# AlibabaResearch/efficientteacher

Measured on AMD Instinct MI355X. Metric: SSOD images/sec (teacher+student step) YOLOv5l 640px, higher is better.
Workload: dtype bf16

## Files before the change

efficientteacher_amd/_lib.py:

```python
import ctypes
import os
from ctypes import c_char_p, c_double, c_float, c_int, c_int64, c_size_t, c_void_p

import torch

_HERE = os.path.dirname(os.path.abspath(__file__))
LIB_PATH = os.environ.get("ET_HIP_LIB") or os.path.join(_HERE, "libet_hip.so")

ET_F32, ET_BF16, ET_F16 = 0, 1, 2

P = c_void_p
SIGNATURES = {
    "et_build_arch": (c_char_p, []),
    "et_abi_version": (c_int, []),
    "et_nms_ssod_workspace_bytes": (c_int, [c_int, c_int, ctypes.POINTER(c_size_t)]),
    "et_nms_workspace_bytes": (c_int, [c_int, c_int, c_int, c_int, c_int, ctypes.POINTER(c_size_t)]),
    "et_nms": (c_int, [P, c_int, c_int, c_int, c_float, c_float, c_int, c_int, ctypes.c_uint64, ctypes.c_uint64, c_int,
                       c_float, c_int, P, P, P, P, P, c_size_t, P]),
    "et_nms_ssod": (c_int, [P, c_int, c_int, c_int, c_float, c_float, c_int, c_int, P, P, P, P, P, c_size_t, P]),
    "et_val_match": (c_int, [P, c_int, P, c_int, c_int, P, c_int, P, c_int, c_int, P, c_int, c_int, c_int, c_int64, c_int64,
                             P, P, P, P, P, P]),
    "et_val_confusion": (c_int, [P, c_int, P, c_int, c_int, P, c_int, P, c_int, c_int, c_float, c_float, c_int, c_int, P, P]),
    "et_val_predn": (c_int, [P, c_int, P, c_int, c_int, P, c_int, c_int, c_int, P, P, P]),
    "et_val_ap_workspace_bytes": (c_int, [c_int, ctypes.POINTER(c_size_t)]),
# ... 37 lines not shown
                              c_size_t, P]),
    "et_bn_act_bwd_from_partials": (c_int, [P, c_int, P, c_int, P, c_int, c_int, c_int, c_int, P, P, P, P, P, c_int, P, P, P,
                                            P, c_int, P, P]),
    "et_act_bwd": (c_int, [P, c_int, P, c_int, P, c_int, c_int, c_int, c_int, c_int, P]),
    "et_pack_input": (c_int, [P, P, c_int, c_int, c_int, c_int, c_int, P]),
    "et_pack_input_u8": (c_int, [P, P, c_int, c_int, c_int, c_int, c_int, c_float, P]),
    "et_maxpool5_fwd": (c_int, [P, c_int, P, c_int, P, c_int, c_int, c_int, c_int, c_int, P]),
    "et_maxpool5_bwd": (c_int, [P, c_int, P, P, c_int, P, c_int, c_int, c_int, c_int, c_int, c_int, P]),
    "et_upsample2x_fwd": (c_int, [P, c_int, P, c_int, c_int, c_int, c_int, c_int, c_int, P]),
    "et_upsample2x_bwd": (c_int, [P, c_int, P, c_int, c_int, c_int, c_int, c_int, c_int, c_int, P]),
    "et_strong_view_u8": (c_int, [P, P, c_int, c_int, c_int, P, P, P, P, c_int, P]),
    "et_mosaic4_u8": (c_int, [P, P, c_int, c_int, c_int, P]),
    "et_pseudo_label_transform": (c_int, [P, P, P, c_int, c_int, c_int, c_int, c_int, P, P, P]),
    "et_score_log_append": (c_int, [P, P, c_int, c_int, P, P, P, c_int64, P]),
    "et_yolo_loss": (c_int, [P, P]),
    "et_ota_workspace_bytes": (c_int, [c_int, c_int, c_int, c_int, ctypes.POINTER(c_size_t)]),
    "et_ota_assign": (c_int, [P, P, c_float, c_int, P, P, P]),
    "et_select_targets": (c_int, [P, P, c_int, P, P, c_int, c_int, P, P]),
    "et_scale_cast": (c_int, [P, P, c_int, c_int64, c_float, P, P]),
    "et_domain_focal": (c_int, [P, c_int, c_int, c_int64, c_int, c_float, P, c_int, P, P]),
    "et_scale_inplace": (c_int, [P, c_int, c_int64, c_float, P, P]),
    "et_v8_decode": (c_int, [P, c_int, P, c_int, c_int, c_int, c_int, c_int, c_int, c_int, c_float, c_float, P, c_int64, c_int64, P]),
    "et_tal_loss": (c_int, [P, P, P, P, P, P, P, c_int, c_int, c_int, c_int, c_int, c_float, c_float, c_float, P, P, P, P, P]),
    "et_tal_assign_workspace_bytes": (c_int, [c_int, c_int, c_int, ctypes.POINTER(c_size_t)]),
    "et_tal_assign": (c_int, [P, P, P, P, P, P, c_int, c_int, c_int, c_int, c_int, c_float, c_float, c_float, P, P, P, P, P, c_size_t, P]),
    "et_tal_targets_pad": (c_int, [P, c_int, c_int, c_int, c_float, c_float, P, P, P]),
    "et_tal_pseudo_split": (c_int, [P, P, P, P, c_int, c_int, c_int, c_int, c_int, c_int, c_float, c_float, P, P, P, P, P, P, P, P, P]),
    "et_tal_assigned_gt": (c_int, [P, c_int, c_int, c_int, P, P]),
    "et_tal_merge_pseudo": (c_int, [P, P, P, P, P, P, P, P, P, c_int, c_int, c_int, c_int, P, P, P, P]),
}
# ... 132 lines not shown
```

efficientteacher_amd/autograd.py:

```python
import torch
from torch.autograd import Function

from . import ops

ACT_CODE = {"silu": ops.ACT_SILU, "relu": ops.ACT_RELU, "none": ops.ACT_NONE}

FUSE_BN_BWD = True
FUSE_BN_BWD_K = 1
_RS_DGRAD = {}


def _dgrad_on_rs_tile(cs, x):
    key = (tuple(x.shape), x.dtype, cs.cinp, cs.coutp, cs.k, cs.stride, cs.pad)
    r = _RS_DGRAD.get(key)
    if r is None:
        N, H, W, _ = x.shape
        r = _RS_DGRAD[key] = cs.stride == 1 and ops.kernel_name("dgrad_full", x.dtype, N, H, W, cs.cinp, cs.coutp, cs.k, cs.stride,
                                                               cs.pad).startswith("conv_gemm_rs_kernel")
    return r


def _fuse_into(cs, bn, x=None):
    if bn is None:
        return None
# ... 274 lines not shown
        dx = None
        if ctx.x_needs_grad:
            wf = cs1.w_lp.as_strided((2 * c, 1, 1, cs1.cinp), (cs1.cinp, cs1.cinp, cs1.cinp, 1), cs1.w_lp.storage_offset())
            dx = ops.conv2d_dgrad(dy, ops.weight_transpose(wf), (x.shape[1], x.shape[2]), 1, 0)
        return (dx,) + (None,) * 11


class _GradDst:

    def __init__(self, p):
        self.shape, self.stride, self.dtype, self.device = tuple(p.shape), tuple(p.stride()), p.dtype, p.device
        self.span = ops._flat_span(p)
        self.buf = None
        self.written = [False, False]

    def flat(self, half, n):
        if self.buf is None:
            self.buf = torch.empty(self.span, dtype=self.dtype, device=self.device)
        cut = n * self.stride[0]
        self.written[half] = True
        return self.buf[:cut] if half == 0 else self.buf[cut:]


class BatchSplitFn(Function):
    @staticmethod
    def forward(ctx, p, n, holder):
        ctx.n, ctx.holder = n, holder
        return p[:n], p[n:]

    @staticmethod
# ... 203 lines not shown
```

efficientteacher_amd/csrc/loss.hip:

```cpp
#include "et_device.h"
#include "../../include/et_hip.h"

#define LOSS_NPASS 4
#define LOSS_MAXL 4

struct LossLevel {
    const void* p;
    float* dp;
    unsigned long long* tobj;
    long long sb, sa, sy, sx;
    int ny, nx;
    float anchors[3][2];
    float balance;
};

struct LossArgs {
    int dtype, B, na, nc, no, NT, nl;
    float anchor_t, gr, cp, cn, cls_pw, obj_pw, box_w, obj_w, cls_w;
    int pass_mask;
    int ignore_obj;
    float* balance_dev;
    int ssi;
    float fl_gamma;
    int obj_ch;
// ... 222 lines not shown
                }
#pragma unroll
                for (int i = 0; i < 4; ++i) sg[i] = 1.0f / (1.0f + expf(-lg[i]));
                pb[0] = sg[0] * 2.f - 0.5f; pb[1] = sg[1] * 2.f - 0.5f;
                const float tw = sg[2] * 2, th = sg[3] * 2;
                pb[2] = tw * tw * L.anchors[r.a][0]; pb[3] = th * th * L.anchors[r.a][1];
                const float ciou = ciou_fwd_bwd(pb, r.tb, g);
                box_sum = 1.0f - ciou;
                const float wgt = -A.box_w / npos;
                atomicAdd(L.dp + off + 0, wgt * g[0] * 2.f * sg[0] * (1.f - sg[0]));
                atomicAdd(L.dp + off + 1, wgt * g[1] * 2.f * sg[1] * (1.f - sg[1]));
                atomicAdd(L.dp + off + 2, wgt * g[2] * L.anchors[r.a][0] * 8.f * sg[2] * sg[2] * (1.f - sg[2]));
                atomicAdd(L.dp + off + 3, wgt * g[3] * L.anchors[r.a][1] * 8.f * sg[3] * sg[3] * (1.f - sg[3]));
                if (pass == 0) {
                    const float tv = (1.0f - A.gr) + A.gr * fmaxf(ciou, 0.f);
                    atomicMax(L.tobj + cell, ((unsigned long long)r.seq << 32) | __float_as_uint(tv));
                }
            }
            if (pass == 1) {
                const float tv = A.ignore_obj ? -1.0f : r.score;
                atomicMax(L.tobj + cell, ((unsigned long long)r.seq << 32) | __float_as_uint(tv));
            }
            if (want_cls) {
                do_cls = true;
                cls_off = off;
                cls_c = r.c;
                cls_wgt = A.cls_w / (npos * (float)A.nc);
            }
        }
    }
    if (A.dtype == ET_F32) cls_sum += loss_class_walk<float>(A, L, do_cls, cls_off, cls_c, cls_wgt);
    else if (A.dtype == ET_F16) cls_sum += loss_class_walk<et_f16>(A, L, do_cls, cls_off, cls_c, cls_wgt);
    else cls_sum += loss_class_walk<uint16_t>(A, L, do_cls, cls_off, cls_c, cls_wgt);
    box_sum = et_wave_sum(box_sum);
    cls_sum = et_wave_sum(cls_sum);
    if ((threadIdx.x & 63) == 0) {
        if (box_sum != 0.f) atomicAdd(A.acc + level * 16 + ACC_BOX0 + pass, box_sum);
        if (cls_sum != 0.f) atomicAdd(A.acc + level * 16 + ACC_CLS0 + pass, cls_sum);
    }
}

__global__ __launch_bounds__(256) void loss_obj_kernel(LossArgs A, LossLevels Ls, int mode) {
    const int level = blockIdx.z;
    const LossLevel& L = Ls.l[level];
    const float fixed_n = Ls.fixed_n[level];
    const unsigned ncell = (unsigned)A.B * A.na * L.ny * L.nx;
    const unsigned plane = (unsigned)L.nx * L.ny;
    float lsum = 0.f, cnt = 0.f;
    const float n = (mode == 1) ? (fixed_n > 0.f ? fixed_n : A.acc[level * 16 + ACC_OBJN]) : 1.f;
    const float bal = (mode == 1) ? (A.balance_dev ? A.balance_dev[level] : L.balance) : 0.f;
    if (blockIdx.x * 256u >= ncell) return;
    for (unsigned i = blockIdx.x * 256u + threadIdx.x; i < ncell; i += gridDim.x * 256u) {
        const unsigned long long w = L.tobj[i];
        const float t = w ? __uint_as_float((unsigned)(w & 0xffffffffull)) : 0.0f;
        if (t >= 0.0f) {
            cnt += 1.f;
            if (mode == 1) {
                const unsigned q = i / plane, rem = i - q * plane;
                const unsigned gj = rem / (unsigned)L.nx, gi = rem - gj * (unsigned)L.nx;
                const unsigned b = q / (unsigned)A.na, a = q - b * (unsigned)A.na;
                const long long off = (long long)b * L.sb + (long long)a * L.sa + (long long)gj * L.sy + (long long)gi * L.sx + A.obj_ch;
                const float x = ld_logit(L.p, A.dtype, off);
                float g;
                lsum += focal_bce_logits(x, t, A.obj_pw, A.fl_gamma, g);
                L.dp[off] += g * (A.obj_w * bal / n);
            }
        }
    }
    __shared__ float red[2][4];
    lsum = et_wave_sum(lsum);
    cnt = et_wave_sum(cnt);
    if ((threadIdx.x & 63) == 0) { red[0][threadIdx.x >> 6] = lsum; red[1][threadIdx.x >> 6] = cnt; }
    __syncthreads();
    if (threadIdx.x == 0) {
        if (mode == 1) atomicAdd(A.acc + level * 16 + ACC_OBJ, red[0][0] + red[0][1] + red[0][2] + red[0][3]);
        else atomicAdd(A.acc + level * 16 + ACC_OBJN, red[1][0] + red[1][1] + red[1][2] + red[1][3]);
    }
}

__global__ void loss_finalize_kernel(LossArgs A, float b0, float b1, float b2, float b3, long long n0, long long n1,
// ... 13 lines not shown
                if ((p == 0 || p == 3) && A.nc > 1) lcls += a[ACC_CLS0 + p] / (n * (float)A.nc);
            }
        }
        const float nobj = A.ignore_obj ? a[ACC_OBJN] : (float)ncell[l];
        const float obji = a[ACC_OBJ] / nobj;
        lobj += obji * (A.balance_dev ? A.balance_dev[l] : bal[l]);
        if (A.balance_dev && A.ssi >= 0) A.balance_dev[l] = A.balance_dev[l] * 0.9999f + 0.0001f / obji;
    }
    if (A.balance_dev && A.ssi >= 0) {
        const float ref = A.balance_dev[A.ssi];
        for (int l = 0; l < A.nl; ++l) A.balance_dev[l] = A.balance_dev[l] / ref;
    }
    lbox *= A.box_w; lobj *= A.obj_w; lcls *= A.cls_w;
    out[0] = lbox; out[1] = lobj; out[2] = lcls;
    out[3] = (lbox + lobj + lcls) * (float)A.B;
}

#define OTA_K 13

struct OtaArgs {
    LossArgs A;
    LossLevel L[LOSS_MAXL];
    float stride[LOSS_MAXL];
    float img_size;
    int topk;
    int* order;
    int* istart;
    float* cbox;
    float* cs0;
    long long* coff;
// ... 243 lines not shown
    if (d->dtype != ET_F32 && d->dtype != ET_BF16 && d->dtype != ET_F16) return -2;
    const long long nq = (long long)d->nl * 5 * d->na * d->NT;
    if (nq >= (1ll << 31)) return -2;
    if (d->NT == 0) return 0;
    hipStream_t s = (hipStream_t)stream;
    OtaArgs O;
    LossArgs& A = O.A;
    A.dtype = d->dtype; A.B = d->B; A.na = d->na; A.nc = d->nc; A.no = d->nc + 5; A.NT = d->NT; A.nl = d->nl;
    A.anchor_t = d->anchor_t; A.gr = d->gr; A.cp = d->cp; A.cn = d->cn; A.cls_pw = d->cls_pw; A.obj_pw = d->obj_pw;
    A.box_w = d->box_w; A.obj_w = d->obj_w; A.cls_w = d->cls_w;
    A.pass_mask = 1; A.ignore_obj = 0; A.obj_ch = 4; A.ota_match = nullptr; A.fl_gamma = 0.f; A.balance_dev = nullptr; A.ssi = -1;
    A.tgt = d->targets; A.acc = nullptr;
    for (int l = 0; l < LOSS_MAXL; ++l) {
        LossLevel& L = O.L[l];
        O.stride[l] = 0.f;
        L.p = nullptr; L.dp = nullptr; L.tobj = nullptr; L.sb = L.sa = L.sy = L.sx = 0; L.ny = L.nx = 1; L.balance = 0.f;
        for (int a = 0; a < 3; ++a) L.anchors[a][0] = L.anchors[a][1] = 1.f;
        if (l >= d->nl) continue;
        const et_loss_level* e = &d->level[l];
        if (!e->p) return -1;
        L.p = e->p; L.sb = e->sb; L.sa = e->sa; L.sy = e->sy; L.sx = e->sx; L.ny = e->ny; L.nx = e->nx;
        for (int a = 0; a < d->na; ++a) { L.anchors[a][0] = e->anchors[2 * a]; L.anchors[a][1] = e->anchors[2 * a + 1]; }
        O.stride[l] = strides[l];
    }
    O.img_size = img_size; O.topk = top_k;
    char* w = (char*)workspace;
    O.coff = (long long*)w;  w += sizeof(long long) * nq;
    O.cbox = (float*)w;      w += sizeof(float) * 4 * nq;
    O.cs0 = (float*)w;       w += sizeof(float) * nq;
    O.cimg = (int*)w;        w += sizeof(int) * nq;
    O.cnt = (int*)w;         w += sizeof(int) * nq;
// ... 49 lines not shown
    const float f = dev_scale ? scale * dev_scale[0] : scale;
    if (i < n) d[i] = et_elem<T>::st(s[i] * f);
}

template <typename T = uint16_t>
__global__ __launch_bounds__(256) void scale_cast_bf16_vec8_kernel(const float* __restrict__ s, T* __restrict__ d, long long n8,
                                                                   float scale, const float* __restrict__ dev_scale) {
    const long long i = (long long)blockIdx.x * 256 + threadIdx.x;
    if (i >= n8) return;
    const float f = dev_scale ? scale * dev_scale[0] : scale;
    const float4 a = *(const float4*)(s + i * 8), b = *(const float4*)(s + i * 8 + 4);
    *(uint4*)(d + i * 8) = make_uint4(et_lp<T>::pack(a.x * f, a.y * f), et_lp<T>::pack(a.z * f, a.w * f), et_lp<T>::pack(b.x * f, b.y * f),
                                      et_lp<T>::pack(b.z * f, b.w * f));
}

extern "C" int et_yolo_loss(const et_loss_desc* d, et_stream_t stream) {
    if (!d || !d->targets || !d->acc_ws || !d->out) return -1;
    if (d->nl < 1 || d->nl > LOSS_MAXL || d->na < 1 || d->na > 3 || d->nc < 1 || d->NT < 0) return -2;
    if ((long long)5 * d->na * d->NT >= (1ll << 27)) return -2;
    hipStream_t s = (hipStream_t)stream;
    LossArgs A;
    A.dtype = d->dtype; A.B = d->B; A.na = d->na; A.nc = d->nc; A.no = d->nc + 5; A.NT = d->NT; A.nl = d->nl;
    A.anchor_t = d->anchor_t; A.gr = d->gr; A.cp = d->cp; A.cn = d->cn; A.cls_pw = d->cls_pw; A.obj_pw = d->obj_pw;
    A.box_w = d->box_w; A.obj_w = d->obj_w; A.cls_w = d->cls_w;
    A.pass_mask = d->pass_mask; A.ignore_obj = d->ignore_obj;
    A.ota_match = d->ota_match; A.obj_ch = d->obj_channel ? d->obj_channel : 4;
    A.fl_gamma = d->fl_gamma;
    A.balance_dev = d->balance_dev; A.ssi = d->balance_dev ? d->autobalance_ssi : -1;
    if (A.balance_dev && A.ssi >= A.nl) return -2;
    if (A.obj_ch < 4 || A.obj_ch >= A.no) return -2;
    A.tgt = d->targets; A.acc = d->acc_ws;
    if (A.dtype != ET_F32 && A.dtype != ET_BF16 && A.dtype != ET_F16) return -2;
    (void)hipMemsetAsync(d->acc_ws, 0, sizeof(float) * 16 * LOSS_MAXL, s);
    float bal[4] = {0, 0, 0, 0};
    long long ncell[4] = {0, 0, 0, 0};
    LossLevels Ls;
    long long ob_max = 1;
    for (int l = 0; l < d->nl; ++l) {
        const et_loss_level* e = &d->level[l];
        if (!e->p || !e->dp || !e->tobj_ws) return -1;
        LossLevel& L = Ls.l[l];
        L.p = e->p; L.dp = e->dp; L.tobj = (unsigned long long*)e->tobj_ws;
        L.sb = e->sb; L.sa = e->sa; L.sy = e->sy; L.sx = e->sx; L.ny = e->ny; L.nx = e->nx;
        for (int a = 0; a < d->na; ++a) { L.anchors[a][0] = e->anchors[2 * a]; L.anchors[a][1] = e->anchors[2 * a + 1]; }
        L.balance = e->balance;
        bal[l] = e->balance;
        ncell[l] = (long long)d->B * d->na * e->ny * e->nx;
        if (ncell[l] >= (1ll << 31)) return -2;
        Ls.fixed_n[l] = d->ignore_obj ? 0.f : (float)ncell[l];
        const long long ob = et_cdiv(ncell[l], 256);
        ob_max = ob > ob_max ? ob : ob_max;
        (void)hipMemsetAsync(e->tobj_ws, 0, (size_t)ncell[l] * 8, s);
    }
    for (int l = d->nl; l < LOSS_MAXL; ++l) { Ls.l[l] = Ls.l[0]; Ls.fixed_n[l] = 0.f; }
    const int nslot = 5 * d->na * d->NT;
    if (nslot > 0) {
        const dim3 grid((nslot + 255) / 256, LOSS_NPASS, d->nl);
        hipLaunchKernelGGL(loss_count_kernel, grid, dim3(256), 0, s, A, Ls);
        hipLaunchKernelGGL(loss_pos_kernel, grid, dim3(256), 0, s, A, Ls);
    }
    const dim3 og((unsigned)(ob_max < 512 ? ob_max : 512), 1, d->nl);
    if (d->ignore_obj) hipLaunchKernelGGL(loss_obj_kernel, og, dim3(256), 0, s, A, Ls, 0);
    hipLaunchKernelGGL(loss_obj_kernel, og, dim3(256), 0, s, A, Ls, 1);
    hipLaunchKernelGGL(loss_finalize_kernel, dim3(1), dim3(64), 0, s, A, bal[0], bal[1], bal[2], bal[3], ncell[0], ncell[1],
                       ncell[2], ncell[3], d->out);
    ET_CHECK_LAUNCH();
    return 0;
}

extern "C" int et_select_targets(const double* targets9, const uint8_t* valid, int N, const double* thr_low,
                                 const double* thr_high, int nc, int with_obj, float* table, et_stream_t stream) {
    if (!targets9 || !thr_low || !thr_high || !table) return -1;
    if (N < 0 || nc < 1) return -2;
    if (N == 0) return 0;
    hipLaunchKernelGGL(select_targets_kernel, dim3((N + 255) / 256), dim3(256), 0, (hipStream_t)stream, targets9, valid, N,
                       thr_low, thr_high, nc, with_obj, table);
    ET_CHECK_LAUNCH();
    return 0;
}

// ... 83 lines not shown
```

efficientteacher_amd/models/loss/loss.py:

```python
import torch

from ... import ops
from ...utils.torch_utils import is_parallel


def smooth_BCE(eps=0.1):
    return 1.0 - 0.5 * eps, 0.5 * eps


class YoloLossFn(torch.autograd.Function):

    @staticmethod
    def forward(ctx, table, hp, anchors_host, balance, *p):
        hp = dict(hp)
        ctx.grad_dst = hp.pop("grad_dst", None) or [None] * len(p)
        ota = hp.pop("ota", None)
        if ota is None:
            out, dps = ops.yolo_loss(list(p), table, anchors_host, balance, **hp)
        else:
            pl = list(p)
            match = ops.ota_assign(pl, table, anchors_host, ota["strides"], nc=hp["nc"], anchor_t=hp["anchor_t"],
                                   top_k=ota["top_k"], img_size=ota["img_size"])
            o1, dps = ops.yolo_loss(pl, table, anchors_host, balance, ota_match=match, obj_channel=hp["nc"] + 4, **hp)
            o2, dps = ops.yolo_loss(pl, table, anchors_host, balance, dps=dps, **hp)
            out = o1 + o2
        ctx.dps = dps
        ctx.meta = [(pi.shape, pi.stride(), pi.dtype) for pi in p]
        ctx.bs = p[0].shape[0]
        ctx.mark_non_differentiable()
        return out

    @staticmethod
    def backward(ctx, gout):
        g3 = gout[3:4].contiguous().float()
        grads = []
        for dp, (shape, stride, dtype), dst in zip(ctx.dps, ctx.meta, ctx.grad_dst):
            out = None
            if dst is not None:
                holder, half, n = dst
                flat = holder.flat(half, n)
                if flat.numel() == dp.numel() and holder.dtype == dtype:
                    out = flat
            g = ops.scale_cast(dp, dtype, scale=float(ctx.bs), dev_scale=g3, out=out)
            grads.append(g.as_strided(shape, stride))
        return (None, None, None, None, *grads)


def _head_of(model):
    return model.module.head if is_parallel(model) else model.head

# ... 81 lines not shown
```

efficientteacher_amd/ops.py:

```python
import torch

from . import _lib
from ._lib import ET_BF16, ET_F16, ET_F32

ACT_NONE, ACT_SILU, ACT_RELU = 0, 1, 2


class KernelTimer:

    def __init__(self):
        self.rows = []
        self.shapes = []

    def span(self, tag, flops, launches=1, nbytes=0, shape=None):
        a, b = torch.cuda.Event(enable_timing=True), torch.cuda.Event(enable_timing=True)
        self.rows.append((tag, flops, launches, nbytes, a, b))
        self.shapes.append(shape)
        return a, b

    def summary(self):
        agg = {}
        for tag, fl, n, nb, a, b in self.rows:
            ms = a.elapsed_time(b)
            t = agg.setdefault(tag, dict(ms=0.0, flops=0.0, launches=0, bytes=0.0))
            t["ms"] += ms; t["flops"] += fl; t["launches"] += n; t["bytes"] += nb
        return agg


TIMER = None
SCOPE = None


class FamilyTimer:

    FAMILY = {
        "et_conv2d_fwd": "gather_gemm", "et_conv2d_dgrad": "gather_gemm", "et_conv2d_dgrad_bn": "gather_gemm",
        "et_conv2d_wgrad": "wgrad", "et_conv2d_wgrad_grouped": "wgrad", "et_conv2d_stem_u8_fwd": "gather_gemm", "et_conv2d_stem_u8_wgrad": "wgrad",
        "et_bn_finalize": "bn", "et_bn_act_fwd": "bn", "et_bn_act_fwd_sharded": "bn", "et_bn_act_bwd_sharded": "bn", "et_bn_act_bwd": "bn", "et_bn_act_bwd_from_partials": "bn", "et_act_bwd": "bn",
        "et_nms": "nms_loss_pl", "et_nms_ssod": "nms_loss_pl", "et_detect_decode": "nms_loss_pl", "et_pseudo_label_transform": "nms_loss_pl",
        "et_select_targets": "nms_loss_pl", "et_yolo_loss": "nms_loss_pl", "et_ota_assign": "nms_loss_pl", "et_score_log_append": "nms_loss_pl",
        "et_scale_cast": "nms_loss_pl", "et_domain_focal": "nms_loss_pl", "et_scale_inplace": "nms_loss_pl", "et_v8_decode": "nms_loss_pl",
        "et_tal_loss": "nms_loss_pl", "et_tal_assign": "nms_loss_pl", "et_colsum": "nms_loss_pl", "et_tal_pseudo_split": "nms_loss_pl", "et_tal_targets_pad": "nms_loss_pl",
        "et_tal_assigned_gt": "nms_loss_pl", "et_tal_merge_pseudo": "nms_loss_pl",
        "et_sgd_nesterov": "optimizer_ema", "et_sgd_nesterov_dev": "optimizer_ema", "et_adamw": "optimizer_ema", "et_ema_update": "optimizer_ema",
        "et_ema_update_dev": "optimizer_ema", "et_cast_f32_to_lp": "optimizer_ema", "et_scaler_check": "optimizer_ema", "et_scaler_update": "optimizer_ema", "et_weight_transpose": "optimizer_ema",
        "et_weight_transpose_all": "optimizer_ema", "et_bn_eval_affine": "optimizer_ema",
    }

    def __init__(self):
        self.rows = []

    def begin(self, name):
        fam = self.FAMILY.get(name, "pool_upsample_pack")
        if fam == "gather_gemm":
            fam = "gather_gemm_teacher" if SCOPE == "teacher" else "gather_gemm_student"
# ... 836 lines not shown
        assert balance_dev.dtype == torch.float32 and balance_dev.numel() >= len(p) and balance_dev.device == dev
        d.balance_dev = _lib.ptr(balance_dev); d.autobalance_ssi = int(ssi)
    keep, new_dps = [table, acc], []
    for i, pi in enumerate(p):
        _, _, ny, nx, _ = pi.shape
        dp = dps[i] if dps is not None else torch.zeros(_flat_span(pi), dtype=torch.float32, device=dev)
        assert dp.numel() == _flat_span(pi)
        tobj = torch.empty(B * na * ny * nx, dtype=torch.int64, device=dev)
        L = d.level[i]
        L.dp = _lib.ptr(dp); L.tobj_ws = _lib.ptr(tobj)
        new_dps.append(dp); keep.append(tobj)
    _lib.check(lib.et_yolo_loss(ctypes.byref(d), _lib.stream(p[0])), "et_yolo_loss")
    return out, new_dps


def ota_assign(p, table, anchors_host, strides, *, nc, anchor_t, top_k=13, img_size=640.0):
    import ctypes
    lib = _lib.load()
    dev = p[0].device
    B, na, nl, NT = p[0].shape[0], p[0].shape[1], len(p), int(table.shape[0])
    table = table.contiguous()
    hp = dict(nc=nc, anchor_t=anchor_t, gr=1.0, cp=1.0, cn=0.0, cls_pw=1.0, obj_pw=1.0, box_w=0.0, obj_w=0.0, cls_w=0.0)
    d = _loss_desc(p, table, anchors_host, [0.0] * nl, hp, 1, False)
    match = torch.full((nl * 5 * na * NT,), -1, dtype=torch.int32, device=dev)
    if NT == 0:
        return match
    d.targets = _lib.ptr(table)
    nbytes = ctypes.c_size_t(0)
    _lib.check(lib.et_ota_workspace_bytes(B, na, nl, NT, ctypes.byref(nbytes)), "et_ota_workspace_bytes")
    ws = torch.empty(nbytes.value, dtype=torch.uint8, device=dev)
# ... 232 lines not shown
```

efficientteacher_amd/trainer/graph_step.py:

```python
import torch

from .. import ops


class HostStager:

    def __init__(self, n, device, slots=8, dtype=torch.float32):
        self.dev = torch.zeros(n, dtype=dtype, device=device)
        self.host = [torch.zeros(n, dtype=dtype).pin_memory() for _ in range(slots)]
        self.ev = [None] * slots
        self.i = 0

    def push(self, values):
        k = self.i % len(self.host)
        self.i += 1
        if self.ev[k] is not None:
            self.ev[k].synchronize()
        h = self.host[k]
        h.copy_(values if torch.is_tensor(values) else torch.as_tensor(values, dtype=h.dtype))
        self.dev.copy_(h, non_blocking=True)
        e = torch.cuda.Event()
        e.record()
        self.ev[k] = e
        return self.dev
# ... 38 lines not shown
            import torch.distributed as dist
            from ..parallel import FlatDataParallel
            if not (isinstance(t.model, FlatDataParallel) and dist.is_initialized() and dist.get_backend(t.model.pg) == "nccl"):
                return False
        if type(t.compute_loss).__name__ != "ComputeLoss":
            return False
        from ..optim import FlatSGD
        opt = t.optimizer
        if not isinstance(opt, FlatSGD) or opt.first:
            return False
        if targets.shape[0] > self.TARGET_CAPACITY:
            return False
        if self.graph is not None and self._signature(imgs) != self.sig:
            torch.cuda.synchronize(t.device)
            self.graph, self.items = None, None
            self.recaptures += 1
        return True

    def _capture(self, imgs, u_str, u_ori, M_s):
        t = self.t
        dev = t.device
        opt = t.optimizer
        emas = [e for e in (t.ema, t.semi_ema) if e is not None]
        self.hp = HostStager(4 * len(opt.param_groups) + 2 * len(emas), dev)
        opt.hp_dev = self.hp.dev[:4 * len(opt.param_groups)].view(len(opt.param_groups), 4)
        for i, e in enumerate(emas):
            e.d_dev = self.hp.dev[4 * len(opt.param_groups) + 2 * i:4 * len(opt.param_groups) + 2 * i + 2]
        self.emas = emas
        self.s_imgs, self.s_ustr, self.s_uori = imgs, u_str, u_ori
        self.s_M = M_s.to(device=dev, dtype=torch.float64).contiguous()
        self.tbl = HostStager(self.TARGET_CAPACITY * 8, dev, slots=4)
        self.s_table = self.tbl.dev.view(self.TARGET_CAPACITY, 8)
        self.hp.push(self._scalars(advance=False))
        torch.cuda.synchronize(dev)
        g = torch.cuda.CUDAGraph()
        for e in emas:
            e.capturing = True
        t._capturing = True
        opt.capturing = True
        import gc
        gc_was_on = gc.isenabled()
        gc.disable()
        try:
            with torch.cuda.graph(g, capture_error_mode="thread_local" if t.RANK != -1 else "global"):
                self.items = t._train_instance_eager(self.s_imgs, None, None, self.s_ustr, self.s_uori, None, self.s_M, 0,
                                                     sup_table=self.s_table)
        finally:
            if gc_was_on:
                gc.enable()
            t._capturing = False
            opt.capturing = False
            for e in emas:
                e.capturing = False
        self.graph = g
        self.sig = self._signature(imgs)
        self._probe, self._since_capture, self.probe_ms = [], 0, None

    def _check_probe(self):
        t = self.t
        self._probe[-1][1].synchronize()
        ms = sorted(a.elapsed_time(b) for a, b in self._probe)
        self.probe_ms = ms[len(ms) // 2]
        self._probe = []
        eager = t.eager_step_ms()
        if eager is None or self.probe_ms <= self.slow_factor * eager:
            return True
        self.slow_captures += 1
        torch.cuda.synchronize(t.device)
        self.graph, self.items = None, None
        if self.slow_captures >= 2:
            raise SlowReplay(f"captured step replays in {self.probe_ms:.1f} ms, the eager step takes {eager:.1f} ms (twice)")
        self.recaptures += 1
        return True

    def _scalars(self, advance=True):
        vals = self.t.optimizer.hp_values()
        for e in self.emas:
            d = e.advance() if advance else 0.5
            vals += [float(d), float(1. - d)]
        return vals

    def run(self, imgs, targets, u_str, u_ori, M_s, ni):
        t = self.t
        if self.graph is not None and len(self._probe) == self.REPLAY_PROBE:
# ... 40 lines not shown
```

include/et_hip.h:

```cpp
#ifndef ET_HIP_H
#define ET_HIP_H
#include <stddef.h>
#include <stdint.h>

#ifdef __cplusplus
extern "C" {
#endif

typedef void* et_stream_t;

enum { ET_F32 = 0, ET_BF16 = 1, ET_F16 = 2 };

#define ET_ABI_VERSION 9
const char* et_build_arch(void);
int et_abi_version(void);

int et_nms_ssod_workspace_bytes(int B, int A, size_t* bytes );
int et_nms_ssod(const float* pred, int B, int A, int no, float conf_thres, float iou_thres,
                int agnostic, int max_det, float* dets, int* counts, int64_t* keep,
                int* n_candidates, void* workspace, size_t ws_bytes, et_stream_t stream);

int et_nms_workspace_bytes(int B, int A, int no, int multi_label, int max_nms, size_t* bytes );
int et_nms(const float* pred, int B, int A, int no, float conf_thres, float iou_thres, int agnostic,
           int multi_label, uint64_t class_mask_lo, uint64_t class_mask_hi, int max_nms, float max_wh,
           int max_det, float* dets, int* counts, int64_t* keep, int* n_candidates, void* workspace,
           size_t ws_bytes, et_stream_t stream);

int et_val_match(const float* dets, int det_row_stride, const int* counts, int B, int max_det, const float* targets, int NT,
// ... 138 lines not shown
typedef struct {
    int dtype, B, na, nc, NT, nl;
    float anchor_t, gr, cp, cn, cls_pw, obj_pw, box_w, obj_w, cls_w;
    int pass_mask, ignore_obj;
    const float* targets;
    float* acc_ws;
    float* out;
    const int* ota_match;
    int obj_channel;
    float* balance_dev;
    int autobalance_ssi;
    float fl_gamma;
    et_loss_level level[4];
} et_loss_desc;
int et_yolo_loss(const et_loss_desc* desc , et_stream_t stream);
int et_ota_workspace_bytes(int B, int na, int nl, int NT, size_t* bytes);
int et_ota_assign(const et_loss_desc* desc , const float* strides , float img_size, int top_k,
                  void* workspace, int* match, et_stream_t stream);
int et_select_targets(const double* targets9, const uint8_t* valid, int N, const double* thr_low,
                      const double* thr_high, int nc, int with_obj, float* table, et_stream_t stream);
int et_scale_cast(const float* src, void* dst, int dtype, int64_t n, float scale,
                  const float* dev_scale , et_stream_t stream);

int et_domain_focal(const void* feat, int ldf, int dtype, int64_t P, int label, float gscale, void* grad,
                    int ldg, float* loss_sum, et_stream_t stream);
int et_scale_inplace(void* x, int dtype, int64_t n, float alpha, const float* dev_scale ,
                     et_stream_t stream);

int et_v8_decode(const void* reg, int ld_reg, const void* cls, int ld_cls, int dtype, int B, int H, int W, int reg_max, int nc,
                 float stride, float cell_offset, float* out, int64_t A_total, int64_t a_offset, et_stream_t stream);
// ... 26 lines not shown
```

Measured before the change: 1311.

## Use pooled sparse loss workspaces and emit dense grads in backward

Result: no change. 1319, median of 6 (+0.6%).

```diff
diff --git a/efficientteacher_amd/_lib.py b/efficientteacher_amd/_lib.py
--- a/efficientteacher_amd/_lib.py
+++ b/efficientteacher_amd/_lib.py
@@ -75,6 +75,8 @@
     "et_pseudo_label_transform": (c_int, [P, P, P, c_int, c_int, c_int, c_int, c_int, P, P, P]),
     "et_score_log_append": (c_int, [P, P, c_int, c_int, P, P, P, c_int64, P]),
     "et_yolo_loss": (c_int, [P, P]),
+    "et_yolo_loss_ws": (c_int, [P, P, P, P]),
+    "et_yolo_loss_emit": (c_int, [P, P, P, P, c_int, c_float, P, P]),
     "et_ota_workspace_bytes": (c_int, [c_int, c_int, c_int, c_int, ctypes.POINTER(c_size_t)]),
     "et_ota_assign": (c_int, [P, P, c_float, c_int, P, P, P]),
     "et_select_targets": (c_int, [P, P, c_int, P, P, c_int, c_int, P, P]),
diff --git a/efficientteacher_amd/autograd.py b/efficientteacher_amd/autograd.py
--- a/efficientteacher_amd/autograd.py
+++ b/efficientteacher_amd/autograd.py
@@ -312,6 +312,10 @@
         self.buf = None
         self.written = [False, False]
 
+    def span_of(self, half, n):
+        cut = n * self.stride[0]
+        return cut if half == 0 else self.span - cut
+
     def flat(self, half, n):
         if self.buf is None:
             self.buf = torch.empty(self.span, dtype=self.dtype, device=self.device)
diff --git a/efficientteacher_amd/csrc/loss.hip b/efficientteacher_amd/csrc/loss.hip
--- a/efficientteacher_amd/csrc/loss.hip
+++ b/efficientteacher_amd/csrc/loss.hip
@@ -3,11 +3,14 @@
 
 #define LOSS_NPASS 4
 #define LOSS_MAXL 4
+#define LOSS_TOUCHED (1ull << 63)
 
 struct LossLevel {
     const void* p;
     float* dp;
     unsigned long long* tobj;
+    float* gobj;
+    unsigned char* mark;
     long long sb, sa, sy, sx;
     int ny, nx;
     float anchors[3][2];
@@ -260,14 +263,17 @@
                 atomicAdd(L.dp + off + 3, wgt * g[3] * L.anchors[r.a][1] * 8.f * sg[3] * sg[3] * (1.f - sg[3]));
                 if (pass == 0) {
                     const float tv = (1.0f - A.gr) + A.gr * fmaxf(ciou, 0.f);
-                    atomicMax(L.tobj + cell, ((unsigned long long)r.seq << 32) | __float_as_uint(tv));
+                    atomicMax(L.tobj + cell, LOSS_TOUCHED | ((unsigned long long)r.seq << 32) | __float_as_uint(tv));
+                } else {
+                    atomicOr(L.tobj + cell, LOSS_TOUCHED);
                 }
             }
             if (pass == 1) {
                 const float tv = A.ignore_obj ? -1.0f : r.score;
-                atomicMax(L.tobj + cell, ((unsigned long long)r.seq << 32) | __float_as_uint(tv));
+                atomicMax(L.tobj + cell, LOSS_TOUCHED | ((unsigned long long)r.seq << 32) | __float_as_uint(tv));
             }
             if (want_cls) {
+                if (pass == 3) atomicOr(L.tobj + cell, LOSS_TOUCHED);
                 do_cls = true;
                 cls_off = off;
                 cls_c = r.c;
@@ -297,8 +303,14 @@
     const float bal = (mode == 1) ? (A.balance_dev ? A.balance_dev[level] : L.balance) : 0.f;
     if (blockIdx.x * 256u >= ncell) return;
     for (unsigned i = blockIdx.x * 256u + threadIdx.x; i < ncell; i += gridDim.x * 256u) {
-        const unsigned long long w = L.tobj[i];
+        const unsigned long long wt = L.tobj[i];
+        const unsigned long long w = wt & ~LOSS_TOUCHED;
         const float t = w ? __uint_as_float((unsigned)(w & 0xffffffffull)) : 0.0f;
+        if (mode == 1 && L.gobj) {
+            L.mark[i] = wt ? 1 : 0;
+            if (wt) L.tobj[i] = 0ull;
+            if (!(t >= 0.0f)) L.gobj[i] = 0.f;
+        }
         if (t >= 0.0f) {
             cnt += 1.f;
             if (mode == 1) {
@@ -309,7 +321,8 @@
                 const float x = ld_logit(L.p, A.dtype, off);
                 float g;
                 lsum += focal_bce_logits(x, t, A.obj_pw, A.fl_gamma, g);
-                L.dp[off] += g * (A.obj_w * bal / n);
+                if (L.gobj) L.gobj[i] = g * (A.obj_w * bal / n);
+                else L.dp[off] += g * (A.obj_w * bal / n);
             }
         }
     }
@@ -353,6 +366,7 @@
     lbox *= A.box_w; lobj *= A.obj_w; lcls *= A.cls_w;
     out[0] = lbox; out[1] = lobj; out[2] = lcls;
     out[3] = (lbox + lobj + lcls) * (float)A.B;
+    for (int i = 0; i < 16 * LOSS_MAXL; ++i) A.acc[i] = 0.f;
 }
 
 #define OTA_K 13
@@ -626,7 +640,7 @@
     for (int l = 0; l < LOSS_MAXL; ++l) {
         LossLevel& L = O.L[l];
         O.stride[l] = 0.f;
-        L.p = nullptr; L.dp = nullptr; L.tobj = nullptr; L.sb = L.sa = L.sy = L.sx = 0; L.ny = L.nx = 1; L.balance = 0.f;
+        L.p = nullptr; L.dp = nullptr; L.tobj = nullptr; L.gobj = nullptr; L.mark = nullptr; L.sb = L.sa = L.sy = L.sx = 0; L.ny = L.nx = 1; L.balance = 0.f;
         for (int a = 0; a < 3; ++a) L.anchors[a][0] = L.anchors[a][1] = 1.f;
         if (l >= d->nl) continue;
         const et_loss_level* e = &d->level[l];
@@ -706,7 +720,7 @@
                                       et_lp<T>::pack(b.z * f, b.w * f));
 }
 
-extern "C" int et_yolo_loss(const et_loss_desc* d, et_stream_t stream) {
+static int yolo_loss_run(const et_loss_desc* d, float* const* gobj, unsigned char* const* mark, et_stream_t stream) {
     if (!d || !d->targets || !d->acc_ws || !d->out) return -1;
     if (d->nl < 1 || d->nl > LOSS_MAXL || d->na < 1 || d->na > 3 || d->nc < 1 || d->NT < 0) return -2;
     if ((long long)5 * d->na * d->NT >= (1ll << 27)) return -2;
@@ -723,16 +737,16 @@
     if (A.obj_ch < 4 || A.obj_ch >= A.no) return -2;
     A.tgt = d->targets; A.acc = d->acc_ws;
     if (A.dtype != ET_F32 && A.dtype != ET_BF16 && A.dtype != ET_F16) return -2;
-    (void)hipMemsetAsync(d->acc_ws, 0, sizeof(float) * 16 * LOSS_MAXL, s);
+    if (!gobj) (void)hipMemsetAsync(d->acc_ws, 0, sizeof(float) * 16 * LOSS_MAXL, s);
     float bal[4] = {0, 0, 0, 0};
     long long ncell[4] = {0, 0, 0, 0};
     LossLevels Ls;
     long long ob_max = 1;
     for (int l = 0; l < d->nl; ++l) {
         const et_loss_level* e = &d->level[l];
-        if (!e->p || !e->dp || !e->tobj_ws) return -1;
+        if (!e->p || !e->dp || !e->tobj_ws || (gobj && (!gobj[l] || !mark || !mark[l]))) return -1;
         LossLevel& L = Ls.l[l];
-        L.p = e->p; L.dp = e->dp; L.tobj = (unsigned long long*)e->tobj_ws;
+        L.p = e->p; L.dp = e->dp; L.tobj = (unsigned long long*)e->tobj_ws; L.gobj = gobj ? gobj[l] : nullptr; L.mark = gobj ? mark[l] : nullptr;
         L.sb = e->sb; L.sa = e->sa; L.sy = e->sy; L.sx = e->sx; L.ny = e->ny; L.nx = e->nx;
         for (int a = 0; a < d->na; ++a) { L.anchors[a][0] = e->anchors[2 * a]; L.anchors[a][1] = e->anchors[2 * a + 1]; }
         L.balance = e->balance;
@@ -742,7 +756,7 @@
         Ls.fixed_n[l] = d->ignore_obj ? 0.f : (float)ncell[l];
         const long long ob = et_cdiv(ncell[l], 256);
         ob_max = ob > ob_max ? ob : ob_max;
-        (void)hipMemsetAsync(e->tobj_ws, 0, (size_t)ncell[l] * 8, s);
+        if (!gobj) (void)hipMemsetAsync(e->tobj_ws, 0, (size_t)ncell[l] * 8, s);
     }
     for (int l = d->nl; l < LOSS_MAXL; ++l) { Ls.l[l] = Ls.l[0]; Ls.fixed_n[l] = 0.f; }
     const int nslot = 5 * d->na * d->NT;
@@ -756,6 +770,120 @@
     hipLaunchKernelGGL(loss_obj_kernel, og, dim3(256), 0, s, A, Ls, 1);
     hipLaunchKernelGGL(loss_finalize_kernel, dim3(1), dim3(64), 0, s, A, bal[0], bal[1], bal[2], bal[3], ncell[0], ncell[1],
                        ncell[2], ncell[3], d->out);
+    ET_CHECK_LAUNCH();
+    return 0;
+}
+
+extern "C" int et_yolo_loss(const et_loss_desc* d, et_stream_t stream) { return yolo_loss_run(d, nullptr, nullptr, stream); }
+
+extern "C" int et_yolo_loss_ws(const et_loss_desc* d, float* const* gobj, unsigned char* const* mark, et_stream_t stream) {
+    if (!gobj || !mark) return -1;
+    if (d && (d->ota_match || (d->obj_channel && d->obj_channel != 4))) return -2;
+    return yolo_loss_run(d, gobj, mark, stream);
+}
+
+struct EmitLevel {
+    float* dp;
+    const unsigned char* mark;
+    const float* gobj;
+    void* dst;
+    long long npix;
+    int plane, CP;
+};
+struct EmitArgs {
+    EmitLevel l[LOSS_MAXL];
+    int na, no, obj_ch;
+    float scale;
+    const float* dev_scale;
+};
+
+template <typename T> __device__ __forceinline__ void emit_store8(T* d, const float* v) {
+    *(uint4*)d = make_uint4(et_lp<T>::pack(v[0], v[1]), et_lp<T>::pack(v[2], v[3]), et_lp<T>::pack(v[4], v[5]), et_lp<T>::pack(v[6], v[7]));
+}
+template <> __device__ __forceinline__ void emit_store8<float>(float* d, const float* v) {
+    *(float4*)d = make_float4(v[0], v[1], v[2], v[3]);
+    *(float4*)(d + 4) = make_float4(v[4], v[5], v[6], v[7]);
+}
+
+template <typename T>
+__global__ __launch_bounds__(256) void loss_emit_kernel(EmitArgs E) {
+    const EmitLevel& L = E.l[blockIdx.z];
+    const int lpp = L.CP >> 3;
+    const long long nitem = L.npix * lpp;
+    const float f = E.dev_scale ? E.scale * E.dev_scale[0] : E.scale;
+    const int nch = E.na * E.no;
+    for (long long i = (long long)blockIdx.x * 256 + threadIdx.x; i < nitem; i += (long long)gridDim.x * 256) {
+        const long long pix = i / lpp;
+        const int c0 = (int)(i - pix * lpp) * 8;
+        float v[8];
+#pragma unroll
+        for (int k = 0; k < 8; ++k) v[k] = 0.f;
+        if (c0 < nch) {
+            const long long b = pix / L.plane;
+            const long long cell0 = b * E.na * L.plane + (pix - b * L.plane);
+            const int a0 = c0 / E.no;
+            unsigned mk = 0;
+            float go[3];
+            int pos[3];
+#pragma unroll
+            for (int t = 0; t < 3; ++t) {
+                const int a = a0 + t;
+                const bool in = a < E.na && a * E.no < c0 + 8;
+                const long long cell = cell0 + (long long)a * L.plane;
+                const int co = a * E.no + E.obj_ch - c0;
+                const bool have = in && co >= 0 && co < 8;
+                if (in) mk |= L.mark[cell];
+                go[t] = have ? L.gobj[cell] : 0.f;
+                pos[t] = have ? co : -1;
+            }
+            if (mk) {
+                float* row = L.dp + pix * L.CP + c0;
+                const float4 x = *(const float4*)row, y = *(const float4*)(row + 4);
+                v[0] = x.x; v[1] = x.y; v[2] = x.z; v[3] = x.w; v[4] = y.x; v[5] = y.y; v[6] = y.z; v[7] = y.w;
+                *(float4*)row = make_float4(0.f, 0.f, 0.f, 0.f);
+                *(float4*)(row + 4) = make_float4(0.f, 0.f, 0.f, 0.f);
+            }
+#pragma unroll
+            for (int t = 0; t < 3; ++t) {
+#pragma unroll
+                for (int k = 0; k < 8; ++k)
+                    if (pos[t] == k) v[k] = v[k] + go[t];
+            }
+        }
+#pragma unroll
+        for (int k = 0; k < 8; ++k) v[k] = v[k] * f;
+        emit_store8<T>((T*)L.dst + pix * L.CP + c0, v);
+    }
+}
+
+extern "C" int et_yolo_loss_emit(const et_loss_desc* d, const float* const* gobj, const unsigned char* const* mark, void* const* dst,
+                                 int dst_dtype, float scale, const float* dev_scale, et_stream_t stream) {
+    if (!d || !gobj || !mark || !dst) return -1;
+    if (d->nl < 1 || d->nl > LOSS_MAXL || d->na < 1 || d->na > 3 || d->nc < 1 || d->B < 1) return -2;
+    if (dst_dtype != ET_F32 && dst_dtype != ET_BF16 && dst_dtype != ET_F16) return -2;
+    EmitArgs E;
+    E.na = d->na; E.no = d->nc + 5; E.obj_ch = 4; E.scale = scale; E.dev_scale = dev_scale;
+    long long gmax = 1;
+    for (int l = 0; l < d->nl; ++l) {
+        const et_loss_level* e = &d->level[l];
+        if (!e->dp || !gobj[l] || !mark[l] || !dst[l]) return -1;
+        const long long CP = e->sx;
+        if (e->ny < 1 || e->nx < 1 || CP < (long long)E.na * E.no || CP > 2048 || (CP & 7) || e->sa != E.no ||
+            e->sy != (long long)e->nx * CP || e->sb != (long long)e->ny * e->nx * CP) return -2;
+        if ((((uintptr_t)e->dp) | ((uintptr_t)dst[l])) & 15) return -2;
+        EmitLevel& L = E.l[l];
+        L.dp = e->dp; L.mark = mark[l]; L.gobj = gobj[l]; L.dst = dst[l];
+        L.plane = e->ny * e->nx; L.CP = (int)CP; L.npix = (long long)d->B * L.plane;
+        if (L.npix * d->na >= (1ll << 31)) return -2;
+        const long long ng = (L.npix * (CP >> 3) + 255) / 256;
+        gmax = ng > gmax ? ng : gmax;
+    }
+    for (int l = d->nl; l < LOSS_MAXL; ++l) E.l[l] = E.l[0];
+    const dim3 grid((unsigned)(gmax < 4096 ? gmax : 4096), 1, d->nl);
+    hipStream_t s = (hipStream_t)stream;
+    if (dst_dtype == ET_F32) hipLaunchKernelGGL((loss_emit_kernel<float>), grid, dim3(256), 0, s, E);
+    else if (dst_dtype == ET_BF16) hipLaunchKernelGGL((loss_emit_kernel<uint16_t>), grid, dim3(256), 0, s, E);
+    else hipLaunchKernelGGL((loss_emit_kernel<et_f16>), grid, dim3(256), 0, s, E);
     ET_CHECK_LAUNCH();
     return 0;
 }
diff --git a/efficientteacher_amd/models/loss/loss.py b/efficientteacher_amd/models/loss/loss.py
--- a/efficientteacher_amd/models/loss/loss.py
+++ b/efficientteacher_amd/models/loss/loss.py
@@ -15,7 +15,11 @@
         hp = dict(hp)
         ctx.grad_dst = hp.pop("grad_dst", None) or [None] * len(p)
         ota = hp.pop("ota", None)
-        if ota is None:
+        ctx.lease = None
+        if ota is None and ops.emit_layout(p):
+            out, ctx.lease = ops.yolo_loss_ws(list(p), table, anchors_host, balance, **hp)
+            dps = None
+        elif ota is None:
             out, dps = ops.yolo_loss(list(p), table, anchors_host, balance, **hp)
         else:
             pl = list(p)
@@ -34,6 +38,19 @@
     def backward(ctx, gout):
         g3 = gout[3:4].contiguous().float()
         grads = []
+        if ctx.lease is not None:
+            dtype = ctx.meta[0][2]
+            outs = []
+            for n_el, dst in zip(ctx.lease.spans, ctx.grad_dst):
+                out = None
+                if dst is not None:
+                    holder, half, n = dst
+                    if holder.dtype == dtype and holder.span_of(half, n) == n_el:
+                        out = holder.flat(half, n)
+                outs.append(out)
+            flats = ops.yolo_loss_emit(ctx.lease, dtype, scale=float(ctx.bs), dev_scale=g3, outs=outs)
+            grads = [g.as_strided(shape, stride) for g, (shape, stride, _) in zip(flats, ctx.meta)]
+            return (None, None, None, None, *grads)
         for dp, (shape, stride, dtype), dst in zip(ctx.dps, ctx.meta, ctx.grad_dst):
             out = None
             if dst is not None:
diff --git a/efficientteacher_amd/ops.py b/efficientteacher_amd/ops.py
--- a/efficientteacher_amd/ops.py
+++ b/efficientteacher_amd/ops.py
@@ -38,7 +38,7 @@
         "et_conv2d_wgrad": "wgrad", "et_conv2d_wgrad_grouped": "wgrad", "et_conv2d_stem_u8_fwd": "gather_gemm", "et_conv2d_stem_u8_wgrad": "wgrad",
         "et_bn_finalize": "bn", "et_bn_act_fwd": "bn", "et_bn_act_fwd_sharded": "bn", "et_bn_act_bwd_sharded": "bn", "et_bn_act_bwd": "bn", "et_bn_act_bwd_from_partials": "bn", "et_act_bwd": "bn",
         "et_nms": "nms_loss_pl", "et_nms_ssod": "nms_loss_pl", "et_detect_decode": "nms_loss_pl", "et_pseudo_label_transform": "nms_loss_pl",
-        "et_select_targets": "nms_loss_pl", "et_yolo_loss": "nms_loss_pl", "et_ota_assign": "nms_loss_pl", "et_score_log_append": "nms_loss_pl",
+        "et_select_targets": "nms_loss_pl", "et_yolo_loss": "nms_loss_pl", "et_yolo_loss_ws": "nms_loss_pl", "et_yolo_loss_emit": "nms_loss_pl", "et_ota_assign": "nms_loss_pl", "et_score_log_append": "nms_loss_pl",
         "et_scale_cast": "nms_loss_pl", "et_domain_focal": "nms_loss_pl", "et_scale_inplace": "nms_loss_pl", "et_v8_decode": "nms_loss_pl",
         "et_tal_loss": "nms_loss_pl", "et_tal_assign": "nms_loss_pl", "et_colsum": "nms_loss_pl", "et_tal_pseudo_split": "nms_loss_pl", "et_tal_targets_pad": "nms_loss_pl",
         "et_tal_assigned_gt": "nms_loss_pl", "et_tal_merge_pseudo": "nms_loss_pl",
@@ -905,6 +905,158 @@
     return out, new_dps
 
 
+class LossWorkspace:
+
+    def __init__(self, key, dev, spans, cells):
+        self.key = key
+        self.dp = [torch.zeros(n, dtype=torch.float32, device=dev) for n in spans]
+        self.tobj = [torch.zeros(n, dtype=torch.int64, device=dev) for n in cells]
+        self.gobj = [torch.empty(n, dtype=torch.float32, device=dev) for n in cells]
+        self.mark = [torch.empty(n, dtype=torch.uint8, device=dev) for n in cells]
+        self.acc = torch.zeros(64, dtype=torch.float32, device=dev)
+        self.state = "clean"
+        self.pinned = False
+
+    def scrub(self):
+        for t in self.dp + self.tobj + [self.acc]:
+            t.zero_()
+        self.state = "clean"
+
+    def buffers(self):
+        return self.dp + self.tobj + [self.acc]
+
+
+class _LossWorkspacePool:
+
+    def __init__(self):
+        import threading
+        self._free, self._pinned, self._lock = {}, [], threading.Lock()
+        self.capture_owner = None
+
+    def acquire(self, key, dev, spans, cells):
+        with self._lock:
+            lst = self._free.get(key)
+            ws = lst.pop() if lst else None
+        if ws is None:
+            ws = LossWorkspace(key, dev, spans, cells)
+        elif ws.state != "clean":
+            ws.scrub()
+        if dev.type == "cuda" and torch.cuda.is_current_stream_capturing():
+            ws.pinned = True
+            with self._lock:
+                self._pinned.append((self.capture_owner, ws))
+        ws.state = "forward"
+        return ws
+
+    def release(self, ws):
+        if ws.pinned:
+            return
+        with self._lock:
+            self._free.setdefault(ws.key, []).append(ws)
+
+    def unpin(self, owner):
+        with self._lock:
+            mine = [ws for o, ws in self._pinned if o is owner and owner is not None]
+            self._pinned = [(o, ws) for o, ws in self._pinned if not (o is owner and owner is not None)]
+            for ws in mine:
+                ws.pinned, ws.state = False, "clean"
+                self._free.setdefault(ws.key, []).append(ws)
+
+    def clear(self):
+        with self._lock:
+            self._free.clear()
+
+    def free_workspaces(self):
+        with self._lock:
+            return [ws for lst in self._free.values() for ws in lst]
+
+
+LOSS_POOL = _LossWorkspacePool()
+
+
+class LossLease:
+
+    def __init__(self, ws, desc, gobj_arr, mark_arr, spans, keep):
+        self.ws, self.desc, self.gobj_arr, self.mark_arr, self.spans, self.keep = ws, desc, gobj_arr, mark_arr, spans, keep
+        self.emitted, self.redo = False, None
+
+    def __del__(self):
+        try:
+            if self.ws is not None:
+                ws, self.ws = self.ws, None
+                LOSS_POOL.release(ws)
+        except Exception:
+            pass
+
+
+def emit_layout(p):
+    for pi in p:
+        if pi.dim() != 5 or pi.dtype not in (torch.float32, torch.bfloat16, torch.float16) or pi.shape[0] < 1:
+            return False
+        _, na, ny, nx, no = pi.shape
+        sb, sa, sy, sx, sc = pi.stride()
+        if sc != 1 or sa != no or sx % 8 or sx < na * no or sx > 2048 or sy != nx * sx or sb != ny * sy:
+            return False
+    return True
+
+
+def yolo_loss_ws(p, table, anchors_host, balance, *, nc, anchor_t, gr, cp, cn, cls_pw, obj_pw, box_w, obj_w, cls_w,
+                 pass_mask=1, ignore_obj=False, fl_gamma=0.0, balance_dev=None, ssi=-1):
+    import ctypes
+    lib = _lib.load()
+    dev = p[0].device
+    assert emit_layout(p)
+    B, na = p[0].shape[0], p[0].shape[1]
+    table = table.contiguous()
+    hp = dict(nc=nc, anchor_t=anchor_t, gr=gr, cp=cp, cn=cn, cls_pw=cls_pw, obj_pw=obj_pw, box_w=box_w, obj_w=obj_w, cls_w=cls_w,
+              fl_gamma=fl_gamma)
+    d = _loss_desc(p, table, anchors_host, balance, hp, pass_mask, ignore_obj)
+    spans = [_flat_span(pi) for pi in p]
+    cells = [B * na * pi.shape[2] * pi.shape[3] for pi in p]
+    key = (str(dev), na, tuple(spans), tuple(cells), tuple(int(pi.stride(3)) for pi in p))
+    ws = LOSS_POOL.acquire(key, dev, spans, cells)
+    out = torch.empty(8, dtype=torch.float32, device=dev)
+    d.targets = _lib.ptr(table) if table.numel() else _lib.ptr(ws.acc)
+    d.acc_ws = _lib.ptr(ws.acc); d.out = _lib.ptr(out)
+    redo_bal = None
+    if balance_dev is not None:
+        assert balance_dev.dtype == torch.float32 and balance_dev.numel() >= len(p) and balance_dev.device == dev
+        d.balance_dev = _lib.ptr(balance_dev); d.autobalance_ssi = int(ssi)
+        redo_bal = balance_dev.clone() if ssi >= 0 else balance_dev
+    for i in range(len(p)):
+        d.level[i].dp = _lib.ptr(ws.dp[i]); d.level[i].tobj_ws = _lib.ptr(ws.tobj[i])
+    assert all(g.numel() == c and m.numel() == c and t.numel() == c for g, m, t, c in zip(ws.gobj, ws.mark, ws.tobj, cells))
+    gobj = (ctypes.c_void_p * len(p))(*[_lib.ptr(g) for g in ws.gobj])
+    mark = (ctypes.c_void_p * len(p))(*[_lib.ptr(m) for m in ws.mark])
+    lease = LossLease(ws, d, gobj, mark, spans, [table, balance_dev])
+    lease.redo = (list(p), table, anchors_host, balance, dict(hp, pass_mask=pass_mask, ignore_obj=ignore_obj, balance_dev=redo_bal, ssi=-1))
+    _lib.check(lib.et_yolo_loss_ws(ctypes.byref(d), gobj, mark, _lib.stream(p[0])), "et_yolo_loss_ws")
+    return out, lease
+
+
+def yolo_loss_emit(lease, dtype, scale=1.0, dev_scale=None, outs=None):
+    import ctypes
+    if lease.emitted or lease.ws is None:
+        p, table, anchors_host, balance, kw = lease.redo
+        _, again = yolo_loss_ws(p, table, anchors_host, balance, **kw)
+        return yolo_loss_emit(again, dtype, scale=scale, dev_scale=dev_scale, outs=outs)
+    ws, d = lease.ws, lease.desc
+    dev = ws.acc.device
+    dsts = []
+    for i, n in enumerate(lease.spans):
+        o = outs[i] if outs is not None and outs[i] is not None else torch.empty(n, dtype=dtype, device=dev)
+        assert o.dtype == dtype and o.numel() == n and o.is_contiguous() and o.data_ptr() % 16 == 0
+        dsts.append(o)
+    arr = (ctypes.c_void_p * len(dsts))(*[_lib.ptr(o) for o in dsts])
+    lease.emitted = True
+    _lib.check(_lib.load().et_yolo_loss_emit(ctypes.byref(d), lease.gobj_arr, lease.mark_arr, arr, et_dtype(dsts[0]), float(scale),
+                                             _lib.ptr(dev_scale), _lib.stream(dsts[0])), "et_yolo_loss_emit")
+    ws.state = "clean"
+    lease.ws = None
+    LOSS_POOL.release(ws)
+    return dsts
+
+
 def ota_assign(p, table, anchors_host, strides, *, nc, anchor_t, top_k=13, img_size=640.0):
     import ctypes
     lib = _lib.load()
diff --git a/efficientteacher_amd/trainer/graph_step.py b/efficientteacher_amd/trainer/graph_step.py
--- a/efficientteacher_amd/trainer/graph_step.py
+++ b/efficientteacher_amd/trainer/graph_step.py
@@ -76,6 +76,7 @@
         if self.graph is not None and self._signature(imgs) != self.sig:
             torch.cuda.synchronize(t.device)
             self.graph, self.items = None, None
+            ops.LOSS_POOL.unpin(self)
             self.recaptures += 1
         return True
 
@@ -103,11 +104,13 @@
         import gc
         gc_was_on = gc.isenabled()
         gc.disable()
+        ops.LOSS_POOL.capture_owner = self
         try:
             with torch.cuda.graph(g, capture_error_mode="thread_local" if t.RANK != -1 else "global"):
                 self.items = t._train_instance_eager(self.s_imgs, None, None, self.s_ustr, self.s_uori, None, self.s_M, 0,
                                                      sup_table=self.s_table)
         finally:
+            ops.LOSS_POOL.capture_owner = None
             if gc_was_on:
                 gc.enable()
             t._capturing = False
@@ -130,6 +133,7 @@
         self.slow_captures += 1
         torch.cuda.synchronize(t.device)
         self.graph, self.items = None, None
+        ops.LOSS_POOL.unpin(self)
         if self.slow_captures >= 2:
             raise SlowReplay(f"captured step replays in {self.probe_ms:.1f} ms, the eager step takes {eager:.1f} ms (twice)")
         self.recaptures += 1
diff --git a/include/et_hip.h b/include/et_hip.h
--- a/include/et_hip.h
+++ b/include/et_hip.h
@@ -11,7 +11,7 @@
 
 enum { ET_F32 = 0, ET_BF16 = 1, ET_F16 = 2 };
 
-#define ET_ABI_VERSION 9
+#define ET_ABI_VERSION 10
 const char* et_build_arch(void);
 int et_abi_version(void);
 
@@ -180,6 +180,11 @@
     et_loss_level level[4];
 } et_loss_desc;
 int et_yolo_loss(const et_loss_desc* desc , et_stream_t stream);
+int et_yolo_loss_ws(const et_loss_desc* desc , float* const* gobj , unsigned char* const* mark ,
+                    et_stream_t stream);
+int et_yolo_loss_emit(const et_loss_desc* desc , const float* const* gobj , const unsigned char* const* mark ,
+                      void* const* dst , int dst_dtype, float scale, const float* dev_scale ,
+                      et_stream_t stream);
 int et_ota_workspace_bytes(int B, int na, int nl, int NT, size_t* bytes);
 int et_ota_assign(const et_loss_desc* desc , const float* strides , float img_size, int top_k,
                   void* workspace, int* match, et_stream_t stream);
```
